# cvxopt/cvxopt

Hardware: NVIDIA H100
Metric: kkt_factor_solve_gflops_fp64 (higher is better)
Workload: dtype f64

## Files before the change

### cvxopt_b200/csrc/chol.cu

```cuda
#include "common.cuh"
#include <cstdlib>

namespace cvxb {

namespace {

constexpr int PB = 8;
constexpr int SP = 12;
constexpr int LDM = NB + 4;
constexpr int POTF2_SMEM = (NB * LDM + NB * SP + 4 * 80) * 8;
constexpr int kGroup = 4;

template <int PAT>
__device__ __forceinline__ void sym_update(double (&acc)[4][8][2], const double *Ma, const double *Mb) {
#pragma unroll 2
    for (int kk = 0; kk < NB / 4; ++kk) {
        double a[4], bfr[8];
#pragma unroll
        for (int cf = 0; cf < 4; ++cf) a[cf] = -Ma[cf * 8 + kk * 4 * LDM];
#pragma unroll
        for (int rf = 0; rf < 8; ++rf) bfr[rf] = Mb[rf * 8 + kk * 4 * LDM];
#pragma unroll
        for (int mf = 0; mf < 2; ++mf)
#pragma unroll
// ... 281 lines not shown
                    if (phase == 0) {
                        M[(o + ti[u] * 8 + g4) + (o + s + tj[u] * 8 + t4 * 2) * LDM] = c[u][0];
                        M[(o + ti[u] * 8 + g4) + (o + s + tj[u] * 8 + t4 * 2 + 1) * LDM] = c[u][1];
                    } else {
                        M[(o + s + ti[u] * 8 + g4) + (o + tj[u] * 8 + t4 * 2) * LDM] = -c[u][0];
                        M[(o + s + ti[u] * 8 + g4) + (o + tj[u] * 8 + t4 * 2 + 1) * LDM] = -c[u][1];
                    }
                }
            }
            __syncthreads();
        }
    }
    CVXB_STAMP(3)
    for (int e = tid; e < NB * NB; e += 256) {
        int i = e & (NB - 1), k = e >> 7;
        inv[e] = (i >= k) ? M[i + k * LDM] : 0.0;
        invT[e] = (k >= i) ? M[k + i * LDM] : 0.0;
    }
    if (trace && threadIdx.x == 0) {
        unsigned long long t; asm volatile("mov.u64 %0, %%globaltimer;" : "=l"(t)); trace[1] = t;
    }
}

constexpr int TR_CH = 32;
constexpr int TR_R = 5;
constexpr int TRSV_SMEM = (TR_R * NB * TR_CH + 4 * NB + 32 * 129) * 8;

template <bool TRANS, bool VEC>
__global__ void __launch_bounds__(256, 1)
trsv_kernel(int n, const double *__restrict__ L, long long ldl, const double *__restrict__ inv,
            const double *__restrict__ invT, double *b, int *flags, int epoch, long long sL,
            long long sInv, long long sb) {
    extern __shared__ __align__(16) double sm[];
    {
        const long long pb = blockIdx.y;
        L += pb * sL; inv += pb * sInv; invT += pb * sInv; b += pb * sb;
        flags += pb * ((n + NB - 1) / NB);
    }
    double *ring = sm;
    double *xs = ring + TR_R * NB * TR_CH;
    double *part = xs + NB;
    double *tvec = part + 2 * NB;
    double *part2 = tvec + NB;
    const int nblk = (n + NB - 1) / NB;
    const int tid = threadIdx.x, lane = tid & 31, warp = tid >> 5;
    const int bi = TRANS ? (nblk - 1 - (int)blockIdx.x) : (int)blockIdx.x;
    const int i0 = bi * NB;
    const int ni = min(NB, n - i0);
    const int r = tid & (NB - 1), half = tid >> 7;

    double ireg[64];
    {
        const double *ip = (TRANS ? invT : inv) + (long long)bi * NB * NB + r + (long long)(half * 64) * NB;
#pragma unroll
        for (int k = 0; k < 64; ++k) ireg[k] = ip[k * NB];
    }

    const double bown = (tid < ni) ? b[i0 + tid] : 0.0;
    const int nb_dep = TRANS ? (nblk - 1 - bi) : bi;
    const int nchunks = nb_dep * (NB / TR_CH);
    auto issue = [&](int q) {
        const int jj = q / (NB / TR_CH), cc = q % (NB / TR_CH);
        const int j = TRANS ? (nblk - 1 - jj) : jj;
        double *dst = ring + (q % TR_R) * (NB * TR_CH);
        const double *src;
        int nrows, ncols;
        if (!TRANS) { src = L + i0 + (long long)(j * NB + cc * TR_CH) * ldl; nrows = ni; ncols = TR_CH; }
        else { src = L + (long long)j * NB + (long long)(i0 + cc * TR_CH) * ldl; nrows = min(NB, n - j * NB); ncols = min(TR_CH, ni - cc * TR_CH); }
        if (VEC) {
#pragma unroll
            for (int it = 0; it < 8; ++it) {
                const int e = tid + it * 256;
                const int c = e >> 6, rr = (e & 63) * 2;
                const int rem = nrows - rr;
                const int bytes = (c < ncols) ? (rem >= 2 ? 16 : (rem == 1 ? 8 : 0)) : 0;
                cp_async16(dst + c * NB + rr, bytes ? (src + rr + (long long)c * ldl) : L, bytes);
            }
        } else {
#pragma unroll
            for (int it = 0; it < 16; ++it) {
                const int e = tid + it * 256;
                const int c = e >> 7, rr = e & 127;
                const int bytes = (c < ncols && rr < nrows) ? 8 : 0;
                cp_async8(dst + c * NB + rr, bytes ? (src + rr + (long long)c * ldl) : L, bytes);
            }
        }
    };
#pragma unroll
    for (int q = 0; q < TR_R - 1; ++q) {
        if (q < nchunks) issue(q);
        cp_async_commit();
    }

    double acc = 0.0;
    double accc[16];
#pragma unroll
    for (int q = 0; q < 16; ++q) accc[q] = 0.0;

    for (int jj = 0; jj < nb_dep; ++jj) {
        const int j = TRANS ? (nblk - 1 - jj) : jj;
        if (tid == 0) while (ld_acquire(flags + j) != epoch) { }
        __syncthreads();
        if (tid < NB) xs[tid] = (j * NB + tid < n) ? __ldcg(b + j * NB + tid) : 0.0;
#pragma unroll
        for (int cc = 0; cc < NB / TR_CH; ++cc) {
            const int q = jj * (NB / TR_CH) + cc;
            cp_async_wait<TR_R - 2>();
            __syncthreads();
            {
                const int nq = q + TR_R - 1;
                if (nq < nchunks) issue(nq);
                cp_async_commit();
            }
            const double *ch = ring + (q % TR_R) * (NB * TR_CH);
            if (!TRANS) {
#pragma unroll
                for (int c = 0; c < 16; ++c)
                    acc += ch[(half * 16 + c) * NB + r] * xs[cc * TR_CH + half * 16 + c];
            } else {
#pragma unroll
                for (int qc = 0; qc < 4; ++qc) {
                    const double *col = ch + (warp * 4 + qc) * NB;
                    double a = 0.0;
#pragma unroll
                    for (int rr = 0; rr < 4; ++rr) a += col[lane + rr * 32] * xs[lane + rr * 32];
                    accc[cc * 4 + qc] += a;
                }
            }
        }
    }
    cp_async_wait<0>();
    __syncthreads();
    if (!TRANS) {
        part[half * NB + r] = acc;
        __syncthreads();
        if (tid < NB) tvec[tid] = (tid < ni) ? (bown - part[tid] - part[NB + tid]) : 0.0;
        __syncthreads();
    } else {
#pragma unroll
        for (int q = 0; q < 16; ++q) {
            const int c = (q >> 2) * TR_CH + warp * 4 + (q & 3);
            part2[lane * 129 + c] = accc[q];
        }
        __syncthreads();
        if (tid < NB) {
            double sacc = 0.0;
#pragma unroll 8
            for (int l = 0; l < 32; ++l) sacc += part2[l * 129 + tid];
            tvec[tid] = (tid < ni) ? (bown - sacc) : 0.0;
        }
        __syncthreads();
    }
    double a2 = 0.0;
#pragma unroll
    for (int k = 0; k < 64; ++k) a2 += ireg[k] * tvec[half * 64 + k];
    part[half * NB + r] = a2;
    __syncthreads();
    if (tid < ni) b[i0 + tid] = part[tid] + part[NB + tid];
    __threadfence();
    __syncthreads();
    if (tid == 0) st_release(flags + bi, epoch);
}

std::atomic<int> g_trsv_epoch{0};

__global__ void __launch_bounds__(256)
transpose_panel_kernel(const double *__restrict__ W, long long ldw, int rows, double *__restrict__ WT, long long ldt) {
    __shared__ double t[32][33];
    const int r0 = blockIdx.x * 32, k0 = blockIdx.y * 32, tx = threadIdx.x, ty = threadIdx.y;
#pragma unroll
    for (int i = ty; i < 32; i += 8)
        if (r0 + tx < rows) t[i][tx] = W[r0 + tx + (long long)(k0 + i) * ldw];
    __syncthreads();
#pragma unroll
    for (int i = ty; i < 32; i += 8)
        if (r0 + i < rows) WT[k0 + tx + (long long)(r0 + i) * ldt] = t[tx][i];
}

}

int chol_work_create(CholWork &w) {
    int least = 0, greatest = 0;
    CVXB_CUDA(cudaDeviceGetStreamPriorityRange(&least, &greatest));
    CVXB_CUDA(cudaStreamCreateWithPriority(&w.panel_stream, cudaStreamNonBlocking, greatest));
// ... 307 lines not shown
```

### cvxopt_b200/csrc/cone.cu

```cuda
#include "cone.cuh"

namespace cvxb {

int ConeLayout::init(const cvxb_dims *dims) {
    if (!dims || dims->mnl < 0 || dims->ml < 0 || dims->nq < 0 || dims->ns < 0) {
        set_error("dims: negative dimension");
        return CVXB_E_ARG;
    }
    mnl = dims->mnl; ml = dims->ml; nq = dims->nq; ns = dims->ns;
    q.assign(dims->q, dims->q + nq);
    s.assign(dims->s, dims->s + ns);
    sumq = sums = sums2 = sump = maxs = 0;
    q_off.resize(nq); v_off.resize(nq); s_off.resize(ns); s_poff.resize(ns); r_off.resize(ns);
    for (int k = 0; k < nq; ++k) {
        if (q[k] < 1) { set_error("dims['q'] entries must be >= 1"); return CVXB_E_ARG; }
        q_off[k] = sumq; v_off[k] = sumq; sumq += q[k];
    }
    for (int k = 0; k < ns; ++k) {
        if (s[k] < 0) { set_error("dims['s'] entries must be >= 0"); return CVXB_E_ARG; }
        s_off[k] = sums2; s_poff[k] = sump; r_off[k] = sums2;
        sums += s[k]; sums2 += s[k] * s[k]; sump += s[k] * (s[k] + 1) / 2;
        if (s[k] > maxs) maxs = s[k];
    }
    cdim = mnl + ml + sumq + sums2;
// ... 172 lines not shown
    const int warp = threadIdx.x >> 5, lane = threadIdx.x & 31;
    const long long c = (long long)blockIdx.x * 8 + warp;
    if (c >= ncols) return;
    const long long pb = blockIdx.y;
    A += pb * bs.sA; x += pb * bs.sx; y += pb * bs.sy;
    if (HAS_W) w += pb * bs.sw;
    const double *a = A + c * lda;
    double s0 = 0, s1 = 0, s2 = 0, s3 = 0;
    int k = 0;
    if (VEC) {
        const double2 *a2 = reinterpret_cast<const double2 *>(a);
        const double2 *x2 = reinterpret_cast<const double2 *>(x);
        const double2 *w2 = reinterpret_cast<const double2 *>(w);
        const int n2 = nrows >> 1;
        int k2 = lane;
        for (; k2 + 96 < n2; k2 += 128) {
            double2 v0 = a2[k2], v1 = a2[k2 + 32], v2 = a2[k2 + 64], v3 = a2[k2 + 96];
            double2 u0 = x2[k2], u1 = x2[k2 + 32], u2 = x2[k2 + 64], u3 = x2[k2 + 96];
            if (HAS_W) {
                double2 q0 = w2[k2], q1 = w2[k2 + 32], q2 = w2[k2 + 64], q3 = w2[k2 + 96];
                u0.x *= q0.x; u0.y *= q0.y; u1.x *= q1.x; u1.y *= q1.y;
                u2.x *= q2.x; u2.y *= q2.y; u3.x *= q3.x; u3.y *= q3.y;
            }
            s0 += v0.x * u0.x; s0 += v0.y * u0.y;
            s1 += v1.x * u1.x; s1 += v1.y * u1.y;
            s2 += v2.x * u2.x; s2 += v2.y * u2.y;
            s3 += v3.x * u3.x; s3 += v3.y * u3.y;
        }
        for (; k2 < n2; k2 += 32) {
            double2 v0 = a2[k2], u0 = x2[k2];
            if (HAS_W) { double2 q0 = w2[k2]; u0.x *= q0.x; u0.y *= q0.y; }
            s0 += v0.x * u0.x; s0 += v0.y * u0.y;
        }
        k = n2 * 2 + lane;
    } else {
        k = lane;
    }
    for (; k < nrows; k += 32) s1 += a[k] * (HAS_W ? w[k] * x[k] : x[k]);
    double s = warp_sum((s0 + s1) + (s2 + s3));
    if (lane == 0) y[c] = (beta == 0.0) ? alpha * s : alpha * s + beta * y[c];
}

constexpr int GN_CH = 128;
__global__ void __launch_bounds__(256)
gemv_n_partial_kernel(int nrows, int ncols, const double *__restrict__ A, long long lda,
                      const double *__restrict__ x, double *ws, GemvBatch bs, long long sws) {
    __shared__ double xs[GN_CH];
    A += (long long)blockIdx.z * bs.sA; x += (long long)blockIdx.z * bs.sx;
    ws += (long long)blockIdx.z * sws;
    const int c0 = blockIdx.y * GN_CH;
    const int nc = min(GN_CH, ncols - c0);
    if (threadIdx.x < GN_CH) xs[threadIdx.x] = (threadIdx.x < nc) ? x[c0 + threadIdx.x] : 0.0;
    __syncthreads();
    const long long k = (long long)blockIdx.x * 256 + threadIdx.x;
    if (k >= nrows) return;
    const double *a = A + k + (long long)c0 * lda;
    double s0 = 0, s1 = 0, s2 = 0, s3 = 0;
    int c = 0;
    for (; c + 3 < nc; c += 4) {
        s0 += a[(long long)c * lda] * xs[c];
        s1 += a[(long long)(c + 1) * lda] * xs[c + 1];
        s2 += a[(long long)(c + 2) * lda] * xs[c + 2];
        s3 += a[(long long)(c + 3) * lda] * xs[c + 3];
    }
    for (; c < nc; ++c) s0 += a[(long long)c * lda] * xs[c];
    ws[(long long)blockIdx.y * nrows + k] = (s0 + s1) + (s2 + s3);
}
__global__ void gemv_n_reduce_kernel(int nrows, int nchunks, const double *ws, const double *w,
                                     double alpha, double beta, double *y, GemvBatch bs,
                                     long long sws) {
    const long long k = (long long)blockIdx.x * blockDim.x + threadIdx.x;
    if (k >= nrows) return;
    ws += (long long)blockIdx.y * sws; y += (long long)blockIdx.y * bs.sy;
    if (w) w += (long long)blockIdx.y * bs.sw;
    double s = 0.0;
    for (int ch = 0; ch < nchunks; ++ch) s += ws[(long long)ch * nrows + k];
    if (w) s *= w[k];
    y[k] = (beta == 0.0) ? alpha * s : alpha * s + beta * y[k];
}

__global__ void transpose_kernel(const double *src, long long lds, double *dst, long long ldd,
                                 int rows, int cols, long long ssrc, long long sdst) {
    __shared__ double t[32][33];
    src += blockIdx.z * ssrc; dst += blockIdx.z * sdst;
    const int tx = threadIdx.x & 31, ty = threadIdx.x >> 5;
    const int r0 = blockIdx.x * 32, c0 = blockIdx.y * 32;
    for (int cc = ty; cc < 32; cc += 8) {
        int r = r0 + tx, c = c0 + cc;
        t[cc][tx] = (r < rows && c < cols) ? src[r + (long long)c * lds] : 0.0;
    }
    __syncthreads();
    for (int rr = ty; rr < 32; rr += 8) {
        int c = c0 + tx, r = r0 + rr;
        if (r < rows && c < cols) dst[c + (long long)r * ldd] = t[tx][rr];
    }
}

__global__ void vec_mul_kernel(int n, const double *a, const double *b, double *out) {
    int i = blockIdx.x * blockDim.x + threadIdx.x;
    if (i < n) out[i] = a[i] * b[i];
}
// ... 166 lines not shown
```

### cvxopt_b200/csrc/cone.cuh

```cuda
#pragma once
#include "common.cuh"
#include <vector>

namespace cvxb {

struct ConeLayout {
    int mnl = 0, ml = 0, nq = 0, ns = 0;
    std::vector<int> q, s;
    int sumq = 0, sums = 0, sums2 = 0, sump = 0, maxs = 0;
    int cdim = 0, cdim_pckd = 0;
    std::vector<int> q_off;
    std::vector<int> v_off;
    std::vector<int> s_off;
    std::vector<int> s_poff;
    std::vector<int> r_off;
    int *d_q = nullptr, *d_qoff = nullptr, *d_voff = nullptr;
    int *d_s = nullptr, *d_soff = nullptr, *d_spoff = nullptr, *d_roff = nullptr;
    ConeLayout() = default;
    ConeLayout(const ConeLayout &) = delete;
    ConeLayout &operator=(const ConeLayout &) = delete;
    ~ConeLayout();
    int init(const cvxb_dims *dims);
};

// ... 22 lines not shown
int pack_s(const ConeLayout &c, const double *src, long long lds, double *dst, long long ldd,
           int xc, bool vector_mode, cudaStream_t st);
int unpack_s(const ConeLayout &c, const double *src, long long lds, double *dst, long long ldd,
             int xc, cudaStream_t st);

struct GemvBatch {
    int batch = 1;
    long long sA = 0, sw = 0, sx = 0, sy = 0;
};
int gemv_t(int nrows, int ncols, const double *A, long long lda, const double *w, const double *x,
           double alpha, double beta, double *y, cudaStream_t st,
           const GemvBatch &bs = GemvBatch());
int gemv_n_chunks(int ncols);
int gemv_n(int nrows, int ncols, const double *A, long long lda, const double *w, const double *x,
           double alpha, double beta, double *y, double *ws, cudaStream_t st,
           const GemvBatch &bs = GemvBatch());
int vec_mul(int n, const double *a, const double *b, double *out, cudaStream_t st);
int vec_axpby(int n, double alpha, const double *x, double beta, double *y, cudaStream_t st);
int symmetrize_lower(int n, double *A, long long lda, int batch, long long stride, cudaStream_t st);
int transpose_copy(const double *src, long long lds, double *dst, long long ldd, int rows, int cols,
                   cudaStream_t st, int batch = 1, long long ssrc = 0, long long sdst = 0);

#ifdef __CUDACC__
struct WarpTeam {
    int rank;
    static constexpr int size = 32;
    __device__ __forceinline__ double sum(double v) const { return warp_sum(v); }
    __device__ __forceinline__ void sync() const { __syncwarp(); }
};
struct CtaTeam {
    int rank, size;
    double *sh;
    __device__ __forceinline__ double sum(double v) const { return block_sum(v, sh); }
    __device__ __forceinline__ void sync() const { __syncthreads(); }
};
#define TEAM_FOR(i, t, i0, m) _Pragma("unroll 1") for (int i = (i0) + (t).rank; i < (m); i += (t).size)

template <class Team>
__device__ __forceinline__ void q_scale(const Team &t, const double *v, double beta, const double *x, double *y, int m,
                                        bool inverse) {
    double w = 0.0;
    TEAM_FOR(i, t, 0, m) {
        double xi = x[i];
        if (inverse && i == 0) xi = -xi;
        w += v[i] * xi;
    }
// ... 266 lines not shown
```

### cvxopt_b200/csrc/kkt_api.cu

```cuda
#include "cone.cuh"
#include <cstdlib>
#include <cstdarg>
#include <map>
#include <unordered_map>
#include <mutex>
#include <iterator>

namespace cvxb {

static thread_local std::string g_err;
std::atomic<unsigned long long> g_launches{0};
std::atomic<unsigned long long> g_device_bytes{0};


namespace {
struct TmpCache {
    std::mutex mu;
    std::multimap<size_t, void *> free_[64];
    std::unordered_map<void *, std::pair<size_t, int>> live;
    size_t cached = 0, cap = 0;
    bool cap_set = false;
};
TmpCache &tmpc() { static TmpCache *c = new TmpCache; return *c; }
size_t tmp_round(size_t b) { return b <= 4096 ? 4096 : (b + 65535) & ~(size_t)65535; }
// ... 236 lines not shown
            CVXB_TRY(dmma_gemm(g, st));
        }
    }
    return 0;
}

}

namespace {
int kkt_check_args(cvxb_kkt **out, int n, int p, const double *A, int lda) {
    if (!out) { set_error("kkt_create: out is NULL"); return CVXB_E_ARG; }
    *out = nullptr;
    if (n < 0 || p < 0) { set_error("kkt_create: negative size"); return CVXB_E_ARG; }
    if (p > 0 && (!A || lda < p)) { set_error("kkt_create: A must be p x n with lda >= p"); return CVXB_E_ARG; }
    if (p > n) { set_error("kkt_create: Rank(A) < p (p > n)"); return CVXB_E_ARG; }
    return 0;
}

int kkt_open(std::unique_ptr<cvxb_kkt> &k, int n, int p, const cvxb_dims *dims, int device) {
    CVXB_TRY(check_device(device));
    k.reset(new cvxb_kkt());
    k->device = device; k->n = n; k->p = p;
    k->i8_mode = ozaki_mode();
    CVXB_TRY(k->cone.init(dims));
    CVXB_CUDA(cudaStreamCreateWithFlags(&k->st, cudaStreamNonBlocking));
    for (cudaEvent_t *e : {&k->e0, &k->e1, &k->e2, &k->e3, &k->t0, &k->t1, &k->m0, &k->m1})
        CVXB_CUDA(cudaEventCreate(e));
    CVXB_TRY(chol_work_create(k->cw));
    return 0;
}

int kkt_alloc(cvxb_kkt *k, const double *A, int lda, int space) {
    const ConeLayout &c = k->cone;
    const int n = k->n, p = k->p;
    const size_t nn = (size_t)(n > 0 ? n : 1);
    CVXB_TRY(k->Kmat.alloc((size_t)kkt_ldk(k) * nn));
    const int nblk = (n + NB - 1) / NB + 1;
    CVXB_TRY(k->inv.alloc((size_t)2 * nblk * NB * NB));
    k->nrest = c.mnl + c.sumq + c.sump;
    if (k->nrest > 0) {
        k->ldgs = (k->nrest + 1) & ~1;
        CVXB_TRY(k->Gs.alloc((size_t)k->ldgs * nn));
    }
    if (c.sums2 > 0) {
        CVXB_TRY(k->Gunp.alloc((size_t)c.sums2 * nn));
        size_t per_col = (size_t)2 * c.maxs * c.maxs;
// ... 3 lines not shown
        if (want > cap) want = (cap / per_col ? cap / per_col : 1) * per_col;
        CVXB_TRY(k->swork.alloc(want));
    }
    if (c.mnl > 0) CVXB_TRY(k->Dfbuf.alloc((size_t)c.mnl * nn));
    if (p > 0) {
        k->lda_eq = (p + 1) & ~1;
        k->ldas = (n + 1) & ~1;
        k->ldkp = (p + 1) & ~1;
        CVXB_TRY(k->Aeq.alloc((size_t)k->lda_eq * nn));
        CVXB_TRY(k->Asct.alloc((size_t)k->ldas * p));
        CVXB_TRY(k->Kp.alloc((size_t)k->ldkp * p));
        CVXB_TRY(k->invp.alloc((size_t)2 * ((p + NB - 1) / NB + 1) * NB * NB));
        CVXB_TRY(k->yd.alloc((size_t)p));
        CVXB_TRY(upload_matrix(k->Aeq.p, k->lda_eq, A, lda, p, n, space, k->st));
    }
    CVXB_TRY(k->W.alloc(c));
    const size_t cd = (size_t)(c.cdim > 0 ? c.cdim : 1);
    CVXB_TRY(k->bzp.alloc(cd));
    CVXB_TRY(k->zin.alloc(cd));
    CVXB_TRY(k->zt.alloc(cd));
    CVXB_TRY(k->xv.alloc(nn));
    CVXB_TRY(k->yv.alloc(cd > nn ? cd : nn));
    CVXB_TRY(k->gemv_ws.alloc(kkt_gemv_ws_doubles(k)));
    CVXB_CUDA(cudaStreamSynchronize(k->st));
    return 0;
}
}

namespace cvxb {
size_t kkt_gemv_ws_doubles(const cvxb_kkt *k) {
    const ConeLayout &c = k->cone;
    const int n = k->n, p = k->p;
    const int rows = k->sp ? c.cdim - c.ml : c.cdim;
    const size_t nn = (size_t)(n > 0 ? n : 1), cd = (size_t)(rows > 0 ? rows : 1);
    size_t w1 = cd * (size_t)gemv_n_chunks(n), w2 = nn * (size_t)gemv_n_chunks(p > 0 ? p : 1);
    const size_t w3 = (size_t)(p > 0 ? p : 1) * (size_t)gemv_n_chunks(n);
    if (w3 > w1) w1 = w3;
    return w1 > w2 ? w1 : w2;
}
}

cvxb_kkt::~cvxb_kkt() {
    if (st) cudaStreamSynchronize(st);
    for (cudaEvent_t e : {e0, e1, e2, e3, t0, t1, m0, m1}) if (e) cudaEventDestroy(e);
    if (st) cudaStreamDestroy(st);
}
// ... 282 lines not shown
        set_error("factor: leading minor of order %d is not positive definite", info);
        return info;
    }
    k->factored = true;
    return 0;
}

int cvxb_kkt_solve(cvxb_kkt *k, double *x, double *y, double *z, int space) {
    if (!k) { set_error("kkt is NULL"); return CVXB_E_ARG; }
    if (!k->factored) { set_error("solve called before a successful factor"); return CVXB_E_ARG; }
    CVXB_CUDA(cudaSetDevice(k->device));
    const ConeLayout &c = k->cone;
    const int n = k->n, p = k->p;
    cudaStream_t st = k->st;
    CVXB_CUDA(cudaEventRecord(k->e0, st));
    double *xd = x, *zd = z, *ydv = y;
    if (p > 0 && !y) { set_error("solve: y is required when p > 0"); return CVXB_E_ARG; }
    if (space != CVXB_DEVICE) {
        CVXB_TRY(xfer_vec(k->xv.p, x, n, CVXB_HOST, true, st));
        CVXB_TRY(xfer_vec(k->zin.p, z, c.cdim, CVXB_HOST, true, st));
        xd = k->xv.p; zd = k->zin.p;
        if (p > 0) { CVXB_TRY(xfer_vec(k->yd.p, y, p, CVXB_HOST, true, st)); ydv = k->yd.p; }
    }
    CVXB_TRY(kkt_pack_bz(k, zd));
    CVXB_TRY(k->method == 1 ? kkt_qr_solve(k, xd, ydv) : chol_solve(k, xd, ydv));
    CVXB_TRY(kkt_unpack_z(k, zd));
    if (space != CVXB_DEVICE) {
        CVXB_TRY(xfer_vec(x, k->xv.p, n, CVXB_HOST, false, st));
        CVXB_TRY(xfer_vec(z, k->zin.p, c.cdim, CVXB_HOST, false, st));
        if (p > 0) CVXB_TRY(xfer_vec(y, k->yd.p, p, CVXB_HOST, false, st));
    }
    CVXB_CUDA(cudaEventRecord(k->e1, st));
    CVXB_CUDA(cudaStreamSynchronize(st));
    float t;
    cudaEventElapsedTime(&t, k->e0, k->e1);
    k->solve_ms = t;
    return 0;
}

int cvxb_kkt_get_L(cvxb_kkt *k, double *L_host, int ldl) {
    if (!k || !L_host || ldl < k->n) { set_error("get_L: bad arguments"); return CVXB_E_ARG; }
    CVXB_CUDA(cudaSetDevice(k->device));
    CVXB_CUDA(cudaMemcpy2D(L_host, (size_t)ldl * sizeof(double), k->Kmat.p, kkt_ldk(k) * sizeof(double),
                           (size_t)k->n * sizeof(double), k->n, cudaMemcpyDeviceToHost));
    return 0;
}

int cvxb_kkt_last_ms(cvxb_kkt *k, double *factor_ms, double *solve_ms) {
    if (!k) return CVXB_E_ARG;
// ... 120 lines not shown
```

### cvxopt_b200/csrc/kkt_internal.cuh

```cuda
#pragma once
#include "cone.cuh"
#include <memory>

using cvxb::ConeLayout;
using cvxb::DevScaling;
using cvxb::CholWork;
using cvxb::DevBuf;

namespace cvxb {
struct QrState {
    int nq = 0;
    DevBuf<double> Q;
    long long ldQ = 0;
    DevBuf<double> R1;
    DevBuf<double> tau;
    DevBuf<double> GsF;
    DevBuf<double> GsQ;
    long long ldf = 0;
    DevBuf<double> Q3t;
    long long ldq = 0;
    DevBuf<double> C[3], inv[3];
    long long ldc = 0;
    int npass = 2;
    DevBuf<double> w, u, vv, xt, ws, norm2;
// ... 34 lines not shown
    std::unique_ptr<cvxb::SparseL> sp;
    DevBuf<double> Hres;
    DevBuf<double> Hbuf;
    DevBuf<double> Kmat;
    DevBuf<double> inv;
    DevBuf<double> Gs;
    long long ldgs = 0;
    int nrest = 0;
    DevBuf<double> Gunp;
    DevBuf<double> Dfbuf;
    DevBuf<double> Aeq;
    long long lda_eq = 0;
    DevBuf<double> Asct;
    long long ldas = 0;
    DevBuf<double> Kp;
    long long ldkp = 0;
    DevBuf<double> invp;
    DevBuf<double> yd;
    bool singular = false;
    bool first_factor = true;
    DevScaling W;
    DevBuf<double> bzp, zin, zt, xv, yv;
    DevBuf<double> gemv_ws;
    DevBuf<double> swork;
    CholWork cw;
    cudaStream_t st = nullptr;
    cudaEvent_t e0 = nullptr, e1 = nullptr, e2 = nullptr, e3 = nullptr, t0 = nullptr, t1 = nullptr;
    cudaEvent_t m0 = nullptr, m1 = nullptr;
    double mma_ms = 0.0;
    double factor_ms = 0, solve_ms = 0, br[3] = {0, 0, 0};
    bool factored = false;
    int i8_mode = 0;
    DevBuf<char> oz_work;
    int syrk_path = 0;
    int method = 0;
    std::unique_ptr<cvxb::QrState> qr;
    std::unique_ptr<cvxb::LdlState> ldl;
    ~cvxb_kkt();
};


namespace cvxb {
int upload_matrix(double *dst, long long ldd, const double *src, long long lds, int rows, int cols, int space,
                  cudaStream_t st);
int xfer_vec(double *dst, const double *src, size_t n, int space, bool to_device, cudaStream_t st);
inline long long kkt_ldk(const cvxb_kkt *k) { long long l = (k->n + 1) & ~1; return l > 2 ? l : 2; }
int kkt_pack_bz(cvxb_kkt *k, const double *zd);
int kkt_unpack_z(cvxb_kkt *k, double *zd);
int kkt_scale_pack_G(cvxb_kkt *k, double *dst, long long ldd);
int kkt_qr_factor(cvxb_kkt *k, const cvxb_scaling *W, int space);
int kkt_qr_solve(cvxb_kkt *k, double *xd, double *yd);
int kkt_qr_setup(cvxb_kkt *k);
int kkt_ldl_factor(cvxb_kkt *k);
int kkt_ldl_solve(cvxb_kkt *k, double *xd, double *yd);
int kkt_ldl_setup(cvxb_kkt *k, double kktreg);
inline const double *kkt_G_qs(const cvxb_kkt *k) {
    return k->sp ? k->Gown.p : k->G + k->cone.mnl + k->cone.ml;
}
int kkt_sparse_load(cvxb_kkt *k, const long long *rowptr, const int *colind, const double *val);
int kkt_sparse_densify(cvxb_kkt *k);
int kkt_sparse_syrk(cvxb_kkt *k, const double *D, long long ldd, const double *w, double *K, long long ldk);
int kkt_sparse_mv(cvxb_kkt *k, bool trans, const double *w, const double *x, double alpha, double beta, double *y);
size_t kkt_gemv_ws_doubles(const cvxb_kkt *k);
}
```

Baseline: 40190.

## Fuse KKT solve into forward and backward persistent kernels with flag-synchronized TRSV

For the linear-cone-only dense case, the pack, G^T gemv, forward triangular solve, backward solve, G gemv and unpack are merged into two kernels. Gemv blocks stream G through a cp.async ring and publish per-block flags, and TRSV blocks consume those flags as they arrive instead of waiting for separate launches. The aim is to cut launch overhead and to overlap the gemv with the dependent triangular-solve chain. It adds spin-wait synchronization between co-resident blocks, an env toggle, and a risk of deadlock if the blocks are not all resident at once.

```diff
diff --git a/cvxopt_b200/csrc/chol.cu b/cvxopt_b200/csrc/chol.cu
--- a/cvxopt_b200/csrc/chol.cu
+++ b/cvxopt_b200/csrc/chol.cu
@@ -1,4 +1,5 @@
 #include "common.cuh"
+#include "trsv.cuh"
 #include <cstdlib>
 
 namespace cvxb {
@@ -327,144 +328,15 @@
     }
 }
 
-constexpr int TR_CH = 32;
-constexpr int TR_R = 5;
-constexpr int TRSV_SMEM = (TR_R * NB * TR_CH + 4 * NB + 32 * 129) * 8;
-
 template <bool TRANS, bool VEC>
 __global__ void __launch_bounds__(256, 1)
 trsv_kernel(int n, const double *__restrict__ L, long long ldl, const double *__restrict__ inv,
             const double *__restrict__ invT, double *b, int *flags, int epoch, long long sL,
             long long sInv, long long sb) {
     extern __shared__ __align__(16) double sm[];
-    {
-        const long long pb = blockIdx.y;
-        L += pb * sL; inv += pb * sInv; invT += pb * sInv; b += pb * sb;
-        flags += pb * ((n + NB - 1) / NB);
-    }
-    double *ring = sm;
-    double *xs = ring + TR_R * NB * TR_CH;
-    double *part = xs + NB;
-    double *tvec = part + 2 * NB;
-    double *part2 = tvec + NB;
-    const int nblk = (n + NB - 1) / NB;
-    const int tid = threadIdx.x, lane = tid & 31, warp = tid >> 5;
-    const int bi = TRANS ? (nblk - 1 - (int)blockIdx.x) : (int)blockIdx.x;
-    const int i0 = bi * NB;
-    const int ni = min(NB, n - i0);
-    const int r = tid & (NB - 1), half = tid >> 7;
-
-    double ireg[64];
-    {
-        const double *ip = (TRANS ? invT : inv) + (long long)bi * NB * NB + r + (long long)(half * 64) * NB;
-#pragma unroll
-        for (int k = 0; k < 64; ++k) ireg[k] = ip[k * NB];
-    }
-
-    const double bown = (tid < ni) ? b[i0 + tid] : 0.0;
-    const int nb_dep = TRANS ? (nblk - 1 - bi) : bi;
-    const int nchunks = nb_dep * (NB / TR_CH);
-    auto issue = [&](int q) {
-        const int jj = q / (NB / TR_CH), cc = q % (NB / TR_CH);
-        const int j = TRANS ? (nblk - 1 - jj) : jj;
-        double *dst = ring + (q % TR_R) * (NB * TR_CH);
-        const double *src;
-        int nrows, ncols;
-        if (!TRANS) { src = L + i0 + (long long)(j * NB + cc * TR_CH) * ldl; nrows = ni; ncols = TR_CH; }
-        else { src = L + (long long)j * NB + (long long)(i0 + cc * TR_CH) * ldl; nrows = min(NB, n - j * NB); ncols = min(TR_CH, ni - cc * TR_CH); }
-        if (VEC) {
-#pragma unroll
-            for (int it = 0; it < 8; ++it) {
-                const int e = tid + it * 256;
-                const int c = e >> 6, rr = (e & 63) * 2;
-                const int rem = nrows - rr;
-                const int bytes = (c < ncols) ? (rem >= 2 ? 16 : (rem == 1 ? 8 : 0)) : 0;
-                cp_async16(dst + c * NB + rr, bytes ? (src + rr + (long long)c * ldl) : L, bytes);
-            }
-        } else {
-#pragma unroll
-            for (int it = 0; it < 16; ++it) {
-                const int e = tid + it * 256;
-                const int c = e >> 7, rr = e & 127;
-                const int bytes = (c < ncols && rr < nrows) ? 8 : 0;
-                cp_async8(dst + c * NB + rr, bytes ? (src + rr + (long long)c * ldl) : L, bytes);
-            }
-        }
-    };
-#pragma unroll
-    for (int q = 0; q < TR_R - 1; ++q) {
-        if (q < nchunks) issue(q);
-        cp_async_commit();
-    }
-
-    double acc = 0.0;
-    double accc[16];
-#pragma unroll
-    for (int q = 0; q < 16; ++q) accc[q] = 0.0;
-
-    for (int jj = 0; jj < nb_dep; ++jj) {
-        const int j = TRANS ? (nblk - 1 - jj) : jj;
-        if (tid == 0) while (ld_acquire(flags + j) != epoch) { }
-        __syncthreads();
-        if (tid < NB) xs[tid] = (j * NB + tid < n) ? __ldcg(b + j * NB + tid) : 0.0;
-#pragma unroll
-        for (int cc = 0; cc < NB / TR_CH; ++cc) {
-            const int q = jj * (NB / TR_CH) + cc;
-            cp_async_wait<TR_R - 2>();
-            __syncthreads();
-            {
-                const int nq = q + TR_R - 1;
-                if (nq < nchunks) issue(nq);
-                cp_async_commit();
-            }
-            const double *ch = ring + (q % TR_R) * (NB * TR_CH);
-            if (!TRANS) {
-#pragma unroll
-                for (int c = 0; c < 16; ++c)
-                    acc += ch[(half * 16 + c) * NB + r] * xs[cc * TR_CH + half * 16 + c];
-            } else {
-#pragma unroll
-                for (int qc = 0; qc < 4; ++qc) {
-                    const double *col = ch + (warp * 4 + qc) * NB;
-                    double a = 0.0;
-#pragma unroll
-                    for (int rr = 0; rr < 4; ++rr) a += col[lane + rr * 32] * xs[lane + rr * 32];
-                    accc[cc * 4 + qc] += a;
-                }
-            }
-        }
-    }
-    cp_async_wait<0>();
-    __syncthreads();
-    if (!TRANS) {
-        part[half * NB + r] = acc;
-        __syncthreads();
-        if (tid < NB) tvec[tid] = (tid < ni) ? (bown - part[tid] - part[NB + tid]) : 0.0;
-        __syncthreads();
-    } else {
-#pragma unroll
-        for (int q = 0; q < 16; ++q) {
-            const int c = (q >> 2) * TR_CH + warp * 4 + (q & 3);
-            part2[lane * 129 + c] = accc[q];
-        }
-        __syncthreads();
-        if (tid < NB) {
-            double sacc = 0.0;
-#pragma unroll 8
-            for (int l = 0; l < 32; ++l) sacc += part2[l * 129 + tid];
-            tvec[tid] = (tid < ni) ? (bown - sacc) : 0.0;
-        }
-        __syncthreads();
-    }
-    double a2 = 0.0;
-#pragma unroll
-    for (int k = 0; k < 64; ++k) a2 += ireg[k] * tvec[half * 64 + k];
-    part[half * NB + r] = a2;
-    __syncthreads();
-    if (tid < ni) b[i0 + tid] = part[tid] + part[NB + tid];
-    __threadfence();
-    __syncthreads();
-    if (tid == 0) st_release(flags + bi, epoch);
+    const long long pb = blockIdx.y;
+    trsv_block<TRANS, VEC>(sm, n, L + pb * sL, ldl, inv + pb * sInv, invT + pb * sInv, b + pb * sb,
+                           flags + pb * ((n + NB - 1) / NB), epoch, (int)blockIdx.x, nullptr, 0);
 }
 
 std::atomic<int> g_trsv_epoch{0};
diff --git a/cvxopt_b200/csrc/cone.cu b/cvxopt_b200/csrc/cone.cu
--- a/cvxopt_b200/csrc/cone.cu
+++ b/cvxopt_b200/csrc/cone.cu
@@ -218,10 +218,7 @@
                 u0.x *= q0.x; u0.y *= q0.y; u1.x *= q1.x; u1.y *= q1.y;
                 u2.x *= q2.x; u2.y *= q2.y; u3.x *= q3.x; u3.y *= q3.y;
             }
-            s0 += v0.x * u0.x; s0 += v0.y * u0.y;
-            s1 += v1.x * u1.x; s1 += v1.y * u1.y;
-            s2 += v2.x * u2.x; s2 += v2.y * u2.y;
-            s3 += v3.x * u3.x; s3 += v3.y * u3.y;
+            gemv_t_step4(s0, s1, s2, s3, v0, v1, v2, v3, u0, u1, u2, u3);
         }
         for (; k2 < n2; k2 += 32) {
             double2 v0 = a2[k2], u0 = x2[k2];
@@ -233,11 +230,9 @@
         k = lane;
     }
     for (; k < nrows; k += 32) s1 += a[k] * (HAS_W ? w[k] * x[k] : x[k]);
-    double s = warp_sum((s0 + s1) + (s2 + s3));
-    if (lane == 0) y[c] = (beta == 0.0) ? alpha * s : alpha * s + beta * y[c];
-}
-
-constexpr int GN_CH = 128;
+    gemv_t_finish(s0, s1, s2, s3, alpha, beta, y + c, lane);
+}
+
 __global__ void __launch_bounds__(256)
 gemv_n_partial_kernel(int nrows, int ncols, const double *__restrict__ A, long long lda,
                       const double *__restrict__ x, double *ws, GemvBatch bs, long long sws) {
@@ -253,12 +248,9 @@
     const double *a = A + k + (long long)c0 * lda;
     double s0 = 0, s1 = 0, s2 = 0, s3 = 0;
     int c = 0;
-    for (; c + 3 < nc; c += 4) {
-        s0 += a[(long long)c * lda] * xs[c];
-        s1 += a[(long long)(c + 1) * lda] * xs[c + 1];
-        s2 += a[(long long)(c + 2) * lda] * xs[c + 2];
-        s3 += a[(long long)(c + 3) * lda] * xs[c + 3];
-    }
+    for (; c + 3 < nc; c += 4)
+        gemv_n_step4(s0, s1, s2, s3, a[(long long)c * lda], a[(long long)(c + 1) * lda], a[(long long)(c + 2) * lda],
+                     a[(long long)(c + 3) * lda], xs + c);
     for (; c < nc; ++c) s0 += a[(long long)c * lda] * xs[c];
     ws[(long long)blockIdx.y * nrows + k] = (s0 + s1) + (s2 + s3);
 }
@@ -269,10 +261,7 @@
     if (k >= nrows) return;
     ws += (long long)blockIdx.y * sws; y += (long long)blockIdx.y * bs.sy;
     if (w) w += (long long)blockIdx.y * bs.sw;
-    double s = 0.0;
-    for (int ch = 0; ch < nchunks; ++ch) s += ws[(long long)ch * nrows + k];
-    if (w) s *= w[k];
-    y[k] = (beta == 0.0) ? alpha * s : alpha * s + beta * y[k];
+    y[k] = gemv_n_reduce_row(ws, nrows, nchunks, k, w, alpha, beta, beta == 0.0 ? 0.0 : y[k]);
 }
 
 __global__ void transpose_kernel(const double *src, long long lds, double *dst, long long ldd,
diff --git a/cvxopt_b200/csrc/cone.cuh b/cvxopt_b200/csrc/cone.cuh
--- a/cvxopt_b200/csrc/cone.cuh
+++ b/cvxopt_b200/csrc/cone.cuh
@@ -68,6 +68,35 @@
                    cudaStream_t st, int batch = 1, long long ssrc = 0, long long sdst = 0);
 
 #ifdef __CUDACC__
+constexpr int GN_CH = 128;
+
+__device__ __forceinline__ void gemv_t_step4(double &s0, double &s1, double &s2, double &s3, double2 v0, double2 v1,
+                                             double2 v2, double2 v3, double2 u0, double2 u1, double2 u2, double2 u3) {
+    s0 += v0.x * u0.x; s0 += v0.y * u0.y;
+    s1 += v1.x * u1.x; s1 += v1.y * u1.y;
+    s2 += v2.x * u2.x; s2 += v2.y * u2.y;
+    s3 += v3.x * u3.x; s3 += v3.y * u3.y;
+}
+__device__ __forceinline__ void gemv_t_finish(double s0, double s1, double s2, double s3, double alpha, double beta,
+                                              double *yc, int lane) {
+    double s = warp_sum((s0 + s1) + (s2 + s3));
+    if (lane == 0) *yc = (beta == 0.0) ? alpha * s : alpha * s + beta * *yc;
+}
+__device__ __forceinline__ void gemv_n_step4(double &s0, double &s1, double &s2, double &s3, double a0, double a1,
+                                             double a2, double a3, const double *xs) {
+    s0 += a0 * xs[0];
+    s1 += a1 * xs[1];
+    s2 += a2 * xs[2];
+    s3 += a3 * xs[3];
+}
+__device__ __forceinline__ double gemv_n_reduce_row(const double *ws, long long nrows, int nchunks, long long k,
+                                                    const double *w, double alpha, double beta, double yk) {
+    double s = 0.0;
+    for (int ch = 0; ch < nchunks; ++ch) s += __ldcg(ws + (long long)ch * nrows + k);
+    if (w) s *= w[k];
+    return (beta == 0.0) ? alpha * s : alpha * s + beta * yk;
+}
+
 struct WarpTeam {
     int rank;
     static constexpr int size = 32;
diff --git a/cvxopt_b200/csrc/kkt_api.cu b/cvxopt_b200/csrc/kkt_api.cu
--- a/cvxopt_b200/csrc/kkt_api.cu
+++ b/cvxopt_b200/csrc/kkt_api.cu
@@ -282,6 +282,8 @@
     k.reset(new cvxb_kkt());
     k->device = device; k->n = n; k->p = p;
     k->i8_mode = ozaki_mode();
+    const char *fused = getenv("CVXB_SOLVE_FUSED");
+    k->solve_fused = !(fused && fused[0] == '0');
     CVXB_TRY(k->cone.init(dims));
     CVXB_CUDA(cudaStreamCreateWithFlags(&k->st, cudaStreamNonBlocking));
     for (cudaEvent_t *e : {&k->e0, &k->e1, &k->e2, &k->e3, &k->t0, &k->t1, &k->m0, &k->m1})
@@ -331,6 +333,8 @@
     CVXB_TRY(k->xv.alloc(nn));
     CVXB_TRY(k->yv.alloc(cd > nn ? cd : nn));
     CVXB_TRY(k->gemv_ws.alloc(kkt_gemv_ws_doubles(k)));
+    if (k->solve_fused && p == 0 && c.mnl == 0 && k->nrest == 0 && c.ml > 0 && !k->sp && n > 0)
+        CVXB_TRY(kkt_solve_fused_alloc(k));
     CVXB_CUDA(cudaStreamSynchronize(k->st));
     return 0;
 }
@@ -659,9 +663,13 @@
         xd = k->xv.p; zd = k->zin.p;
         if (p > 0) { CVXB_TRY(xfer_vec(k->yd.p, y, p, CVXB_HOST, true, st)); ydv = k->yd.p; }
     }
-    CVXB_TRY(kkt_pack_bz(k, zd));
-    CVXB_TRY(k->method == 1 ? kkt_qr_solve(k, xd, ydv) : chol_solve(k, xd, ydv));
-    CVXB_TRY(kkt_unpack_z(k, zd));
+    if (kkt_solve_fused_ok(k)) {
+        CVXB_TRY(kkt_solve_fused(k, xd, zd));
+    } else {
+        CVXB_TRY(kkt_pack_bz(k, zd));
+        CVXB_TRY(k->method == 1 ? kkt_qr_solve(k, xd, ydv) : chol_solve(k, xd, ydv));
+        CVXB_TRY(kkt_unpack_z(k, zd));
+    }
     if (space != CVXB_DEVICE) {
         CVXB_TRY(xfer_vec(x, k->xv.p, n, CVXB_HOST, false, st));
         CVXB_TRY(xfer_vec(z, k->zin.p, c.cdim, CVXB_HOST, false, st));
diff --git a/cvxopt_b200/csrc/kkt_internal.cuh b/cvxopt_b200/csrc/kkt_internal.cuh
--- a/cvxopt_b200/csrc/kkt_internal.cuh
+++ b/cvxopt_b200/csrc/kkt_internal.cuh
@@ -80,6 +80,10 @@
     DevScaling W;
     DevBuf<double> bzp, zin, zt, xv, yv;
     DevBuf<double> gemv_ws;
+    bool solve_fused = true;
+    DevBuf<double> ubuf;
+    DevBuf<int> solve_sync;
+    int solve_epoch = 0, nsm = 0;
     DevBuf<double> swork;
     CholWork cw;
     cudaStream_t st = nullptr;
@@ -120,4 +124,7 @@
 int kkt_sparse_syrk(cvxb_kkt *k, const double *D, long long ldd, const double *w, double *K, long long ldk);
 int kkt_sparse_mv(cvxb_kkt *k, bool trans, const double *w, const double *x, double alpha, double beta, double *y);
 size_t kkt_gemv_ws_doubles(const cvxb_kkt *k);
+bool kkt_solve_fused_ok(const cvxb_kkt *k);
+int kkt_solve_fused_alloc(cvxb_kkt *k);
+int kkt_solve_fused(cvxb_kkt *k, double *xd, double *zd);
 }
diff --git a/cvxopt_b200/csrc/kkt_solve.cu b/cvxopt_b200/csrc/kkt_solve.cu
--- /dev/null
+++ b/cvxopt_b200/csrc/kkt_solve.cu
@@ -0,0 +1,279 @@
+#include "cone.cuh"
+#include "trsv.cuh"
+#include "kkt_internal.cuh"
+
+namespace cvxb {
+namespace {
+
+constexpr int FT_STAGE = 1024 + 128;
+constexpr int FT_S = 10;
+constexpr int BN_S = 12;
+constexpr int BN_ROWS = 512;
+static_assert(FT_S * FT_STAGE * 16 <= TRSV_SMEM, "forward stream ring exceeds the chain's shared memory");
+static_assert(BN_S * 4 * 256 * 16 + NB * 8 + BN_S * 8 + 5 * 4 <= TRSV_SMEM,
+              "backward stream ring exceeds the chain's shared memory");
+
+struct FusedArgs {
+    int n, ml, nS;
+    const double *G; long long ldg;
+    const double *u;
+    const double *di;
+    double *bzp, *z;
+    double *x;
+    const double *L; long long ldl;
+    const double *inv, *invT;
+    int *cflags, *sflags, *scnt, *tcnt;
+    int *work;
+    int epoch;
+    double *ws;
+};
+
+__global__ void pack_l_kernel(int m, const double *__restrict__ z, const double *__restrict__ di, double *bzp,
+                              double *u, int *work) {
+    const int i = blockIdx.x * blockDim.x + threadIdx.x;
+    if (i == 0) *work = 0;
+    if (i >= m) return;
+    const double w = di[i];
+    const double b = z[i] * w;
+    bzp[i] = b;
+    u[i] = b * w;
+}
+
+__global__ void __launch_bounds__(256, 1) solve_fwd_kernel(FusedArgs a) {
+    extern __shared__ __align__(16) double sm[];
+    const int tid = threadIdx.x;
+    if ((int)blockIdx.x >= a.nS) {
+        trsv_block<false, true>(sm, a.n, a.L, a.ldl, a.inv, a.invT, a.x, a.cflags, a.epoch, (int)blockIdx.x - a.nS,
+                                a.sflags, a.epoch);
+        return;
+    }
+    const int warp = tid >> 5, lane = tid & 31;
+    const int n2 = a.ml >> 1;
+    const int N = (n2 - lane - 96 > 0) ? (n2 - lane - 96 + 127) / 128 : 0;
+    const int ngroups = (a.n + 7) / 8;
+    const int ngm = (ngroups > (int)blockIdx.x) ? (ngroups - (int)blockIdx.x + a.nS - 1) / a.nS : 0;
+    const int NT = (n2 - 96 > 0) ? (n2 - 96 + 127) / 128 : 0;
+    double2 *ring = reinterpret_cast<double2 *>(sm);
+    const double2 *u2 = reinterpret_cast<const double2 *>(a.u);
+    int pgi = NT > 0 ? 0 : ngm, pt = 0, ps = 0;
+    auto issue_next = [&]() {
+        if (pgi < ngm) {
+            const long long col = (long long)((int)blockIdx.x + pgi * a.nS) * 8 + warp;
+            const bool ok = col < a.n && pt < N;
+            const double2 *g2 = reinterpret_cast<const double2 *>(a.G + col * a.ldg) + lane + 128 * pt;
+            double2 *d = ring + ps * FT_STAGE + warp * 128 + lane;
+#pragma unroll
+            for (int i = 0; i < 4; ++i) cp_async16(d + i * 32, ok ? g2 + 32 * i : u2, ok ? 16 : 0);
+            if (warp < 4) {
+                const bool oku = pt < N;
+                cp_async16(ring + ps * FT_STAGE + 1024 + warp * 32 + lane, u2 + (oku ? lane + 128 * pt + 32 * warp : 0),
+                           oku ? 16 : 0);
+            }
+            if (++pt == NT) { pt = 0; ++pgi; }
+        }
+        if (++ps == FT_S) ps = 0;
+        cp_async_commit();
+    };
+#pragma unroll
+    for (int q = 0; q < FT_S - 1; ++q) issue_next();
+    int cs = 0;
+    for (int gi = 0; gi < ngm; ++gi) {
+        const long long col = (long long)((int)blockIdx.x + gi * a.nS) * 8 + warp;
+        double s0 = 0, s1 = 0, s2 = 0, s3 = 0;
+        for (int t = 0; t < NT; ++t) {
+            cp_async_wait<FT_S - 2>();
+            __syncthreads();
+            issue_next();
+            if (t < N) {
+                const double2 *d = ring + cs * FT_STAGE + warp * 128 + lane;
+                const double2 *q = ring + cs * FT_STAGE + 1024 + lane;
+                gemv_t_step4(s0, s1, s2, s3, d[0], d[32], d[64], d[96], q[0], q[32], q[64], q[96]);
+            }
+            if (++cs == FT_S) cs = 0;
+        }
+        if (col >= a.n) continue;
+        const double *g = a.G + col * a.ldg;
+        const double2 *g2 = reinterpret_cast<const double2 *>(g);
+        for (int k2 = lane + 128 * N; k2 < n2; k2 += 32) {
+            const double2 v0 = g2[k2], q0 = u2[k2];
+            s0 += v0.x * q0.x; s0 += v0.y * q0.y;
+        }
+        for (int k = n2 * 2 + lane; k < a.ml; k += 32) s1 += g[k] * a.u[k];
+        gemv_t_finish(s0, s1, s2, s3, 1.0, 1.0, a.x + col, lane);
+        if (lane == 0) {
+            __threadfence();
+            const int j = (int)(col / NB);
+            if (atomicAdd(a.scnt + j, 1) == min(NB, a.n - j * NB) - 1) {
+                a.scnt[j] = 0;
+                __threadfence();
+                st_release(a.sflags + j, a.epoch);
+            }
+        }
+    }
+    cp_async_wait<0>();
+}
+
+__global__ void __launch_bounds__(256, 1) solve_bwd_kernel(FusedArgs a) {
+    extern __shared__ __align__(16) double sm[];
+    const int tid = threadIdx.x;
+    const int nblk = (a.n + NB - 1) / NB;
+    if ((int)blockIdx.x < nblk) {
+        trsv_block<true, true>(sm, a.n, a.L, a.ldl, a.inv, a.invT, a.x, a.cflags, a.epoch, (int)blockIdx.x, nullptr,
+                               0);
+        return;
+    }
+    const int ntiles = (a.ml + BN_ROWS - 1) / BN_ROWS;
+    const int nitems = nblk * ntiles;
+    constexpr int NG = GN_CH / 4;
+    double2 *ring = reinterpret_cast<double2 *>(sm);
+    double *xs = sm + BN_S * 4 * 256 * 2;
+    uint64_t *full = reinterpret_cast<uint64_t *>(xs + GN_CH);
+    int *last = reinterpret_cast<int *>(full + BN_S);
+    int *items = last + 1;
+    int pit = 0, pli = 0, pg = 0, ps = 0;
+    auto grab = [&]() {
+        pit = atomicAdd(a.work, 1);
+        items[pli & 3] = pit < nitems ? pit : -1;
+    };
+    if (tid == 0) {
+        for (int q = 0; q < BN_S; ++q) mbar_init(full + q, 1);
+        asm volatile("fence.mbarrier_init.release.cluster;" ::: "memory");
+        grab();
+    }
+    auto issue_next = [&]() {
+        if (tid != 0 || pit >= nitems) return;
+        const int pch = nblk - 1 - pit / ntiles, ptile = pit % ntiles;
+        const long long k0 = (long long)ptile * BN_ROWS;
+        const uint32_t bytes = (uint32_t)min((long long)BN_ROWS, a.ml - k0) * 8u;
+        const int nc = min(GN_CH, a.n - pch * GN_CH);
+        const int ncol = max(0, min(4, nc - pg * 4));
+        double2 *d = ring + ps * 1024;
+        mbar_expect_tx(full + ps, bytes * ncol);
+        for (int i = 0; i < ncol; ++i)
+            bulk_g2s(d + i * 256, a.G + k0 + (long long)(pch * GN_CH + pg * 4 + i) * a.ldg, bytes, full + ps);
+        if (++ps == BN_S) ps = 0;
+        if (++pg == NG) {
+            pg = 0;
+            ++pli;
+            grab();
+        }
+    };
+    for (int q = 0; q < BN_S - 1; ++q) issue_next();
+    __syncthreads();
+    int cs = 0;
+    uint32_t cph = 0;
+    for (int li = 0;; ++li) {
+        const int it = items[li & 3];
+        if (it < 0) break;
+        const int ch = nblk - 1 - it / ntiles, tile = it % ntiles;
+        const int nc = min(GN_CH, a.n - ch * GN_CH);
+        const long long k = (long long)tile * BN_ROWS + 2 * tid;
+        if (tid == 0) while (ld_acquire(a.cflags + ch) != a.epoch) { }
+        __syncthreads();
+        if (tid < GN_CH) xs[tid] = (tid < nc) ? __ldcg(a.x + ch * GN_CH + tid) : 0.0;
+        double s0 = 0, s1 = 0, s2 = 0, s3 = 0, t0 = 0, t1 = 0, t2 = 0, t3 = 0;
+        for (int gq = 0; gq < NG; ++gq) {
+            mbar_wait(full + cs, cph);
+            __syncthreads();
+            issue_next();
+            const double2 *d = ring + cs * 1024 + tid;
+            const int c = gq * 4;
+            if (c + 3 < nc) {
+                const double2 v0 = d[0], v1 = d[256], v2 = d[512], v3 = d[768];
+                gemv_n_step4(s0, s1, s2, s3, v0.x, v1.x, v2.x, v3.x, xs + c);
+                gemv_n_step4(t0, t1, t2, t3, v0.y, v1.y, v2.y, v3.y, xs + c);
+            } else {
+                for (int i = 0; c + i < nc; ++i) {
+                    const double2 v = d[i * 256];
+                    s0 += v.x * xs[c + i];
+                    t0 += v.y * xs[c + i];
+                }
+            }
+            if (++cs == BN_S) { cs = 0; cph ^= 1u; }
+        }
+        if (k < a.ml) {
+            a.ws[(long long)ch * a.ml + k] = (s0 + s1) + (s2 + s3);
+            a.ws[(long long)ch * a.ml + k + 1] = (t0 + t1) + (t2 + t3);
+        }
+        __threadfence();
+        __syncthreads();
+        if (tid == 0) {
+            const int done = atomicAdd(a.tcnt + tile, 1) == nblk - 1;
+            if (done) a.tcnt[tile] = 0;
+            __threadfence();
+            *last = done;
+        }
+        __syncthreads();
+        if (*last && k < a.ml) {
+            for (int r = 0; r < 2; ++r) {
+                const double y = gemv_n_reduce_row(a.ws, a.ml, nblk, k + r, a.di, 1.0, -1.0, a.bzp[k + r]);
+                a.bzp[k + r] = y;
+                a.z[k + r] = y;
+            }
+        }
+    }
+}
+
+DeviceOnce g_fused_attr;
+
+}
+
+bool kkt_solve_fused_ok(const cvxb_kkt *k) {
+    const ConeLayout &c = k->cone;
+    return k->solve_fused && k->ubuf.p && k->method == 0 && k->p == 0 && c.mnl == 0 && k->nrest == 0 && c.ml > 0 && !k->sp &&
+           k->n > 0 && k->G && (uintptr_t)(k->G + c.mnl) % 16 == 0 && k->ldg % 2 == 0 &&
+           c.ml % 2 == 0 && (uintptr_t)k->W.di % 16 == 0 && (uintptr_t)k->bzp.p % 16 == 0 &&
+           (uintptr_t)k->Kmat.p % 16 == 0 && kkt_ldk(k) % 2 == 0;
+}
+
+int kkt_solve_fused_alloc(cvxb_kkt *k) {
+    const int nblk = (k->n + NB - 1) / NB, ntiles = (k->cone.ml + BN_ROWS - 1) / BN_ROWS;
+    CVXB_TRY(k->ubuf.alloc((size_t)k->cone.ml));
+    const size_t nsync = (size_t)3 * nblk + ntiles + 1;
+    CVXB_TRY(k->solve_sync.alloc(nsync));
+    CVXB_CUDA(cudaMemsetAsync(k->solve_sync.p, 0, nsync * sizeof(int), k->st));
+    int nsm = 0;
+    CVXB_CUDA(cudaDeviceGetAttribute(&nsm, cudaDevAttrMultiProcessorCount, k->device));
+    k->nsm = nsm;
+    return 0;
+}
+
+int kkt_solve_fused(cvxb_kkt *k, double *xd, double *zd) {
+    if (unsigned long long bit = g_fused_attr.pending()) {
+        CVXB_CUDA(cudaFuncSetAttribute(solve_fwd_kernel, cudaFuncAttributeMaxDynamicSharedMemorySize, TRSV_SMEM));
+        CVXB_CUDA(cudaFuncSetAttribute(solve_bwd_kernel, cudaFuncAttributeMaxDynamicSharedMemorySize, TRSV_SMEM));
+        g_fused_attr.mark(bit);
+    }
+    const ConeLayout &c = k->cone;
+    const int n = k->n, ml = c.ml;
+    cudaStream_t st = k->st;
+    const int nblk = (n + NB - 1) / NB, ntiles = (ml + BN_ROWS - 1) / BN_ROWS;
+    FusedArgs a;
+    a.n = n; a.ml = ml;
+    a.G = k->G + c.mnl; a.ldg = k->ldg;
+    a.u = k->ubuf.p; a.di = k->W.di;
+    a.bzp = k->bzp.p; a.z = zd; a.x = xd;
+    a.L = k->Kmat.p; a.ldl = kkt_ldk(k);
+    a.inv = k->inv.p; a.invT = k->inv.p + (long long)nblk * NB * NB;
+    a.cflags = k->solve_sync.p; a.sflags = a.cflags + nblk; a.scnt = a.sflags + nblk; a.tcnt = a.scnt + nblk;
+    a.work = a.tcnt + ntiles;
+    a.ws = k->gemv_ws.p;
+    const int free_sm = k->nsm - nblk > k->nsm / 2 ? k->nsm - nblk : k->nsm / 2;
+    const int want = free_sm > 1 ? free_sm : 1;
+    pack_l_kernel<<<(ml + 255) / 256, 256, 0, st>>>(ml, zd, k->W.di, k->bzp.p, k->ubuf.p, a.work);
+    count_launch();
+    CVXB_LAUNCH_CHECK();
+    a.nS = std::min(want, (n + 7) / 8);
+    a.epoch = ++k->solve_epoch;
+    solve_fwd_kernel<<<a.nS + nblk, 256, TRSV_SMEM, st>>>(a);
+    count_launch();
+    CVXB_LAUNCH_CHECK();
+    a.nS = std::min(want + nblk, nblk * ntiles);
+    a.epoch = ++k->solve_epoch;
+    solve_bwd_kernel<<<nblk + a.nS, 256, TRSV_SMEM, st>>>(a);
+    count_launch();
+    CVXB_LAUNCH_CHECK();
+    return 0;
+}
+
+}
diff --git a/cvxopt_b200/csrc/trsv.cuh b/cvxopt_b200/csrc/trsv.cuh
--- /dev/null
+++ b/cvxopt_b200/csrc/trsv.cuh
@@ -0,0 +1,154 @@
+#pragma once
+#include "common.cuh"
+
+namespace cvxb {
+
+constexpr int TR_CH = 32;
+constexpr int TR_R = 5;
+constexpr int TRSV_SMEM = (TR_R * NB * TR_CH + 4 * NB + 32 * 129) * 8;
+
+template <bool TRANS, bool VEC>
+__device__ __forceinline__ void trsv_block(double *sm, int n, const double *__restrict__ L, long long ldl,
+                                           const double *__restrict__ inv, const double *__restrict__ invT,
+                                           double *b, int *flags, int epoch, int blk, const int *own_flag,
+                                           int own_epoch) {
+    double *ring = sm;
+    double *xs = ring + TR_R * NB * TR_CH;
+    double *part = xs + NB;
+    double *tvec = part + 2 * NB;
+    double *part2 = tvec + NB;
+    const int nblk = (n + NB - 1) / NB;
+    const int tid = threadIdx.x, lane = tid & 31, warp = tid >> 5;
+    const int bi = TRANS ? (nblk - 1 - blk) : blk;
+    const int i0 = bi * NB;
+    const int ni = min(NB, n - i0);
+    const int r = tid & (NB - 1), half = tid >> 7;
+
+    double ireg[64];
+    {
+        const double *ip = (TRANS ? invT : inv) + (long long)bi * NB * NB + r + (long long)(half * 64) * NB;
+#pragma unroll
+        for (int k = 0; k < 64; ++k) ireg[k] = ip[k * NB];
+    }
+
+    double bown = (!own_flag && tid < ni) ? b[i0 + tid] : 0.0;
+    bool own_early = false;
+    const int nb_dep = TRANS ? (nblk - 1 - bi) : bi;
+    const int nchunks = nb_dep * (NB / TR_CH);
+    auto issue = [&](int q) {
+        const int jj = q / (NB / TR_CH), cc = q % (NB / TR_CH);
+        const int j = TRANS ? (nblk - 1 - jj) : jj;
+        double *dst = ring + (q % TR_R) * (NB * TR_CH);
+        const double *src;
+        int nrows, ncols;
+        if (!TRANS) { src = L + i0 + (long long)(j * NB + cc * TR_CH) * ldl; nrows = ni; ncols = TR_CH; }
+        else { src = L + (long long)j * NB + (long long)(i0 + cc * TR_CH) * ldl; nrows = min(NB, n - j * NB); ncols = min(TR_CH, ni - cc * TR_CH); }
+        if (VEC) {
+#pragma unroll
+            for (int it = 0; it < 8; ++it) {
+                const int e = tid + it * 256;
+                const int c = e >> 6, rr = (e & 63) * 2;
+                const int rem = nrows - rr;
+                const int bytes = (c < ncols) ? (rem >= 2 ? 16 : (rem == 1 ? 8 : 0)) : 0;
+                cp_async16(dst + c * NB + rr, bytes ? (src + rr + (long long)c * ldl) : L, bytes);
+            }
+        } else {
+#pragma unroll
+            for (int it = 0; it < 16; ++it) {
+                const int e = tid + it * 256;
+                const int c = e >> 7, rr = e & 127;
+                const int bytes = (c < ncols && rr < nrows) ? 8 : 0;
+                cp_async8(dst + c * NB + rr, bytes ? (src + rr + (long long)c * ldl) : L, bytes);
+            }
+        }
+    };
+#pragma unroll
+    for (int q = 0; q < TR_R - 1; ++q) {
+        if (q < nchunks) issue(q);
+        cp_async_commit();
+    }
+
+    double acc = 0.0;
+    double accc[16];
+#pragma unroll
+    for (int q = 0; q < 16; ++q) accc[q] = 0.0;
+
+    for (int jj = 0; jj < nb_dep; ++jj) {
+        const int j = TRANS ? (nblk - 1 - jj) : jj;
+        const bool last = own_flag && jj == nb_dep - 1;
+        if (tid == 0) {
+            while (ld_acquire(flags + j) != epoch) { }
+            if (last) tvec[0] = (ld_acquire(own_flag + bi) == own_epoch) ? 1.0 : 0.0;
+        }
+        __syncthreads();
+        if (tid < NB) xs[tid] = (j * NB + tid < n) ? __ldcg(b + j * NB + tid) : 0.0;
+        if (last && tvec[0] != 0.0) {
+            own_early = true;
+            if (tid < ni) bown = __ldcg(b + i0 + tid);
+        }
+#pragma unroll
+        for (int cc = 0; cc < NB / TR_CH; ++cc) {
+            const int q = jj * (NB / TR_CH) + cc;
+            cp_async_wait<TR_R - 2>();
+            __syncthreads();
+            {
+                const int nq = q + TR_R - 1;
+                if (nq < nchunks) issue(nq);
+                cp_async_commit();
+            }
+            const double *ch = ring + (q % TR_R) * (NB * TR_CH);
+            if (!TRANS) {
+#pragma unroll
+                for (int c = 0; c < 16; ++c)
+                    acc += ch[(half * 16 + c) * NB + r] * xs[cc * TR_CH + half * 16 + c];
+            } else {
+#pragma unroll
+                for (int qc = 0; qc < 4; ++qc) {
+                    const double *col = ch + (warp * 4 + qc) * NB;
+                    double a = 0.0;
+#pragma unroll
+                    for (int rr = 0; rr < 4; ++rr) a += col[lane + rr * 32] * xs[lane + rr * 32];
+                    accc[cc * 4 + qc] += a;
+                }
+            }
+        }
+    }
+    cp_async_wait<0>();
+    if (own_flag && !own_early) {
+        if (tid == 0) while (ld_acquire(own_flag + bi) != own_epoch) { }
+        __syncthreads();
+        if (tid < ni) bown = __ldcg(b + i0 + tid);
+    }
+    __syncthreads();
+    if (!TRANS) {
+        part[half * NB + r] = acc;
+        __syncthreads();
+        if (tid < NB) tvec[tid] = (tid < ni) ? (bown - part[tid] - part[NB + tid]) : 0.0;
+        __syncthreads();
+    } else {
+#pragma unroll
+        for (int q = 0; q < 16; ++q) {
+            const int c = (q >> 2) * TR_CH + warp * 4 + (q & 3);
+            part2[lane * 129 + c] = accc[q];
+        }
+        __syncthreads();
+        if (tid < NB) {
+            double sacc = 0.0;
+#pragma unroll 8
+            for (int l = 0; l < 32; ++l) sacc += part2[l * 129 + tid];
+            tvec[tid] = (tid < ni) ? (bown - sacc) : 0.0;
+        }
+        __syncthreads();
+    }
+    double a2 = 0.0;
+#pragma unroll
+    for (int k = 0; k < 64; ++k) a2 += ireg[k] * tvec[half * 64 + k];
+    part[half * NB + r] = a2;
+    __syncthreads();
+    if (tid < ni) b[i0 + tid] = part[tid] + part[NB + tid];
+    __threadfence();
+    __syncthreads();
+    if (tid == 0) st_release(flags + bi, epoch);
+}
+
+}
```

New measurement: 40500 (median of 6 runs). About the same (+0.8%).
